# Fannovel16/ComfyUI-Frame-Interpolation

Hardware: AMD Instinct MI355X
Metric: interpolated frames/sec/GPU @1080p RIFE4.7 2x (higher is better)
Workload: dtype f32; 1 GPU; RIFE 4.7 2x, 1080x1920 synthetic frame-pair stream, 32 pairs/step/GPU resident in HBM (BASELINE.json configs[1]; SURVEY 8d config 2 clip: 33 frames torch.manual_seed(0) torch.rand); seeded random-init weights; new_frame_collective=none, launch=one process, one GPU

## Files before the change

### comfyui-frame-interpolation_amd/csrc/conv_mfma.hip

```cpp
#include "vfi_common.h"

#include <atomic>

#include <cstdlib>
#include <map>
#include <string>
#include <cstring>

namespace vfi {

typedef float f32x16 __attribute__((ext_vector_type(16)));
typedef float f32x4 __attribute__((ext_vector_type(4)));

template <int STRIDE, int TAPS, int MT, int NT, int WM, int WN, int CK, bool GROUPED, bool EXT>
__global__ __launch_bounds__(256) void conv_mfma_kernel(const ConvArgs a) {
    static_assert(WM * WN == 4, "4 waves per workgroup");
    static_assert(!GROUPED || (WN == 4 && NT == 1 && TAPS == 4), "grouped: one 2x2 tap group per wave column");
    static_assert(TAPS == 9 || TAPS == 4 || TAPS == 1, "tap rectangle 3x3 / 2x2 / 1x1");
    constexpr int KW = TAPS == 9 ? 3 : (TAPS == 4 ? 2 : 1);
    constexpr int SUBS = WM * MT;
    constexpr int SUBX = SUBS >= 2 ? 2 : 1;
    constexpr int SUBY = SUBS / SUBX;
    constexpr int TWO = SUBX * 8, THO = SUBY * 4;
    constexpr int TWI = STRIDE * (TWO - 1) + 3;
// ... 279 lines not shown
    static std::atomic<int> n_of[kMaxDevices];
    int dev = 0;
    if (hipGetDevice(&dev) != hipSuccess || dev < 0 || dev >= kMaxDevices) return 256;
    int n = n_of[dev].load(std::memory_order_relaxed);
    if (!n) {
        hipDeviceProp_t p;
        if (hipGetDeviceProperties(&p, dev) == hipSuccess) n = p.multiProcessorCount;
        if (n <= 0) n = 256;
        n_of[dev].store(n, std::memory_order_relaxed);
    }
    return n;
}

int conv_pick_variant(const ConvArgs& a, int stride, bool grouped) {
    const long px = (long)(a.split_ok ? a.N : 8) * a.Hout * a.Wout;
    if (!grouped && stride == 1 && a.ntaps == 4 && a.tapmask) return kConv2Base + (a.Cin_p % 16 == 0 ? 28 : 26);
    if (!grouped && stride == 2 && a.ntaps == 4) return kConv2Base + (a.Cout_p % 64 == 0 ? 21 : 20);
    if (!grouped && stride == 1 && a.ntaps != 9) {
        const bool big = px * (a.Cout_p / 32) >= 256L * 4 * n_cus_cached();
        if (a.ntaps == 1 && a.Cout_p % 64 == 0 && a.Cin_p % 32 == 0)
            return kConv2Base + (a.Cin_p >= 512 && a.Cout_p % 128 == 0 ? 24 : 23);
        if (a.Cout_p % 64 == 0) return kConv2Base + (a.ntaps == 4 ? (big ? 14 : 15) : (big ? 16 : 17));
        return kConv2Base + (a.ntaps == 4 ? 19 : 18);
    }
    const long cus = n_cus_cached();
    if (grouped) {
        if (a.out_mode == 1 && px >= 250000) return kConv2Base + 11;
        return a.Cin_p % 16 == 0 ? 13 : kConv2Base + 11;
    }
    const bool n3 = a.Cout_p % 96 == 0;
    const bool n2 = a.Cout_p % 64 == 0;
    (void)cus;
    if (stride == 2) {
        if (n2) return kConv2Base + 7;
        if (n3) return kConv2Base + 9;
        return 10;
    }
    if (a.split_ok && (n2 || n3) && px <= 6000) return kConv2Base + 29;
    if (n2) {
        const long big_px = option(kOptM2n2Px);
        if (a.Cout_p == 64 || (big_px >= 0 && px >= big_px)) return kConv2Base + 0;
        return kConv2Base + 2;
    }
    if (n3) return px >= 100000 || a.Cin_p % 16 ? kConv2Base + 3 : 4;
    return a.Cin_p % 16 == 0 && px < 20000 ? 4 : kConv2Base + 13;
}

int conv_launch(const ConvArgs& a, int stride, bool grouped, int variant, hipStream_t s,
                const char* trace_name) {
    if (variant < 0 && grouped && option(kOptGroupedVariant) >= 0) variant = (int)option(kOptGroupedVariant);
    if (variant < 0 && trace_name) variant = variant_override(trace_name);
    if (variant < 0) variant = conv_pick_variant(a, stride, grouped);
    const ConvVariant* vp = conv_variant_lookup(variant);
    VFI_REQUIRE(vp, "conv: bad variant %d", variant);
    const ConvVariant& v = *vp;
    VFI_REQUIRE(v.stride == stride && (v.grouped != 0) == grouped && v.taps == a.ntaps,
                "conv: variant %s does not match stride %d grouped %d taps %d", v.name, stride, (int)grouped,
                a.ntaps);
    VFI_REQUIRE(a.out_mode != 1 || (grouped && a.Cout % 4 == 0 && a.Cout / 4 <= 4 * (a.out_planes ? a.out_planes : 2)),
                "conv: out_mode 1 is for grouped convs whose pixel-shuffled channels fit the planar4 output");
    VFI_REQUIRE(a.out_mode != 2 || grouped, "conv: out_mode 2 is for grouped convs");
    VFI_REQUIRE(a.act != 3 || a.prelu, "conv: act 3 needs per-channel slopes");
    VFI_REQUIRE(a.Cin_p % 8 == 0 && a.Cout_p % 32 == 0 && a.in_cs >= a.Cin_p && a.in_cs % 4 == 0,
                "conv: bad channel padding Cin_p=%d Cout_p=%d in_cs=%d", a.Cin_p, a.Cout_p, a.in_cs);
    VFI_REQUIRE(((uintptr_t)a.in & 15) == 0 && ((uintptr_t)a.w & 15) == 0, "conv: unaligned pointers");
    const char* nm = trace_name ? trace_name : v.name;
// ... 108 lines not shown
```

### comfyui-frame-interpolation_amd/csrc/conv_mfma2.hip

```cpp
#include "vfi_common.h"

#include <atomic>
#include <cstdlib>
#include <map>
#include <mutex>
#include <utility>

namespace vfi {

typedef float f32x16 __attribute__((ext_vector_type(16)));
typedef float f32x4 __attribute__((ext_vector_type(4)));
typedef __attribute__((address_space(3))) void* lds_ptr_t;
typedef const __attribute__((address_space(1))) void* glb_ptr_t;

template <int STRIDE, int TAPS, int MT, int NT, int WM, int WN, int CK, bool GROUPED>
struct Conv2Geom {
    static constexpr int KW = TAPS == 9 ? 3 : (TAPS == 4 ? 2 : 1);
    static constexpr int SUBS = WM * MT;
    static constexpr int SUBX = SUBS >= 16 ? 4 : (SUBS >= 2 ? 2 : 1);
    static constexpr int SUBY = SUBS / SUBX;
    static constexpr int TWO = SUBX * 8, THO = SUBY * 4;
    static constexpr int PADLO = (TAPS == 9 || GROUPED) ? 1 : 0;
    static constexpr int SPAN = (TAPS == 9 || GROUPED) ? 3 : KW;
    static constexpr int TWI = STRIDE * (TWO - 1) + SPAN;
    static constexpr int THI = STRIDE * (THO - 1) + SPAN;
    static constexpr int NPIX = TWI * THI;
    static constexpr int Q = CK / 4;
    static constexpr int C8 = CK / 8;
    static constexpr int NA_INSTR = (NPIX * Q + 63) / 64;
    static constexpr int A_FLOATS = NA_INSTR * 256;
    static constexpr int NGRP = GROUPED ? 4 : 1;
    static constexpr int BN = GROUPED ? 32 : WN * NT * 32;
    static constexpr int NB_INSTR = NGRP * TAPS * C8 * (BN / 32);
    static constexpr int B_FLOATS = NB_INSTR * 256;
    static constexpr int BUF_FLOATS = A_FLOATS + B_FLOATS;
    static constexpr int LDS_BYTES = 2 * BUF_FLOATS * 4;
    static constexpr int NAW = (NA_INSTR + 3) / 4;
    static constexpr int NBW = (NB_INSTR + 3) / 4;
};

template <int STRIDE, int TAPS, int MT, int NT, int WM, int WN, int CK, bool GROUPED, bool EXT, bool MASKED = false>
__global__ __launch_bounds__(256) void conv_mfma2_kernel(const ConvArgs a) {
#if defined(__HIP_DEVICE_COMPILE__)
    using G = Conv2Geom<STRIDE, TAPS, MT, NT, WM, WN, CK, GROUPED>;
    static_assert(WM * WN == 4, "4 waves per workgroup");
    static_assert(!GROUPED || (WN == 4 && NT == 1 && TAPS == 4), "grouped: one 2x2 tap group per wave column");
    constexpr int KW = G::KW, SUBX = G::SUBX, TWO = G::TWO, THO = G::THO, TWI = G::TWI;
    constexpr int Q = G::Q, C8 = G::C8, BN = G::BN;

    extern __shared__ __attribute__((aligned(16))) float smem[];

    const int tid = threadIdx.x;
    const int lane = tid & 63;
    const int wave = __builtin_amdgcn_readfirstlane(tid >> 6);
    const int wm = wave / WN, wn = wave % WN;
    const int half = lane >> 5, l31 = lane & 31;

    const int g = GROUPED ? wn : 0;
    const int cob = blockIdx.y * BN;
    const int co0 = GROUPED ? cob : cob + wn * NT * 32;
    const int cin8 = a.Cin_p >> 3;
    const int tby = GROUPED ? (g >> 1) - 1 : a.tap_y0;
    const int tbx = GROUPED ? (g & 1) - 1 : a.tap_x0;

    const int tiles_per_img = a.tiles_x * a.tiles_y;
    const int T = a.N * tiles_per_img;
    const int pstr = a.in_plane ? 4 : a.in_cs;
    const int qstr = a.in_plane ? a.in_plane : 4;
    const int cadv = a.in_plane ? (CK / 4) * a.in_plane : CK;
    const int img_floats = a.in_plane ? (a.in_cs / 4) * a.in_plane : a.Hin * a.Win * a.in_cs;
    auto decode = [&](int tile, int& n, int& Y0, int& X0) {
        n = tile / tiles_per_img;
        const int trem = tile - n * tiles_per_img;
        const int ty = trem / a.tiles_x;
        Y0 = ty * THO;
        X0 = (trem - ty * a.tiles_x) * TWO;
    };
    auto make_avoff = [&](int Y0, int X0, int(&avoff)[G::NAW]) {
        const int iy0 = STRIDE * Y0 - G::PADLO, ix0 = STRIDE * X0 - G::PADLO;
#pragma unroll
        for (int i = 0; i < G::NAW; ++i) {
            const int j = wave + 4 * i;
            const int idx = j * 64 + lane;
            const int pix = idx / Q, q = idx - pix * Q;
            const int py = pix / TWI, px = pix - py * TWI;
            const int iy = iy0 + py, ix = ix0 + px;
            if (EXT && a.pad_mode) {
                const int cy = pad_index(iy, a.Hin, a.pad_mode), cx = pad_index(ix, a.Win, a.pad_mode);
                avoff[i] = pix < G::NPIX ? ((cy * a.Win + cx) * pstr + q * qstr) * 4 : (int)0x80000000;
            } else {
                const bool ok = pix < G::NPIX && iy >= 0 && iy < a.Hin && ix >= 0 && ix < a.Win;
                avoff[i] = ok ? ((iy * a.Win + ix) * pstr + q * qstr) * 4 : (int)0x80000000;
            }
        }
    };
    auto make_rsrc = [&](int n) {
        return __builtin_amdgcn_make_buffer_rsrc((void*)(a.in + (size_t)n * img_floats), 0, img_floats * 4, 0x00020000);
    };
    const unsigned tmask = MASKED ? a.tapmask[blockIdx.y] : 0xffffu;
    const int tapstride = cin8 * a.Cout_p * 8;
    const int c8stride = a.Cout_p * 8;
    const float* wsrc[G::NBW];
    bool wlive[G::NBW];
#pragma unroll
    for (int i = 0; i < G::NBW; ++i) {
        const int j = wave + 4 * i;
        const int sub = j % (BN / 32);
        const int c8 = (j / (BN / 32)) % C8;
        const int t = (j / (BN / 32) / C8) % TAPS;
        const int gg = j / (BN / 32) / C8 / TAPS;
        wsrc[i] = a.w + (size_t)(gg * TAPS + t) * tapstride + c8 * c8stride + (cob + sub * 32) * 8 + lane * 4;
        wlive[i] = !MASKED || ((tmask >> t) & 1u);
    }
    auto issue = [&](const __amdgpu_buffer_rsrc_t& rsrc, const int(&avoff)[G::NAW], int chunk, int buf) {
        float* abuf = smem + buf * G::BUF_FLOATS;
        float* bbuf = abuf + G::A_FLOATS;
        const int cbyte = chunk * cadv * 4;
#pragma unroll
        for (int i = 0; i < G::NAW; ++i) {
            const int j = wave + 4 * i;
            if (G::NA_INSTR % 4 == 0 || j < G::NA_INSTR)
                __builtin_amdgcn_raw_ptr_buffer_load_lds(rsrc, (lds_ptr_t)(abuf + j * 256), 16, avoff[i] + cbyte, 0, 0, 0);
        }
        const int wadv = chunk * C8 * c8stride;
#pragma unroll
        for (int i = 0; i < G::NBW; ++i) {
            const int j = wave + 4 * i;
            if ((G::NB_INSTR % 4 == 0 || j < G::NB_INSTR) && wlive[i])
                __builtin_amdgcn_global_load_lds((glb_ptr_t)(wsrc[i] + wadv), (lds_ptr_t)(bbuf + j * 256), 16, 0, 0);
        }
    };

    int abase[MT];
#pragma unroll
    for (int mt = 0; mt < MT; ++mt) {
        const int s = wm * MT + mt;
        const int sx = s % SUBX, sy = s / SUBX;
        const int oy = sy * 4 + (l31 >> 3), ox = sx * 8 + (l31 & 7);
        abase[mt] = ((STRIDE * oy + G::PADLO + tby) * TWI + STRIDE * ox + G::PADLO + tbx) * CK + half * 4;
    }
    const int bbase = G::A_FLOATS + (g * TAPS * C8 * BN + (co0 - cob) + l31) * 8 + half * 4;

    float bs[NT], bt[NT];
#pragma unroll
    for (int nt = 0; nt < NT; ++nt) {
        const int co = co0 + nt * 32 + l31;
        bs[nt] = a.bias[g * a.Cout_p + co];
        bt[nt] = a.beta ? a.beta[co] : 1.f;
    }

    int nchunks = a.Cin_p / CK, k0 = 0;
    float* const outp = a.out + (size_t)blockIdx.z * a.split_stride;
    if (a.ksplit > 1) {
        const int per = (nchunks + a.ksplit - 1) / a.ksplit;
        k0 = blockIdx.z * per;
        nchunks = nchunks - k0 < per ? nchunks - k0 : per;
    }

    int tile = blockIdx.x;
    if (tile >= T) return;
    int n, Y0, X0, avoff[G::NAW];
    decode(tile, n, Y0, X0);
    make_avoff(Y0, X0, avoff);
    __amdgpu_buffer_rsrc_t rsrc = make_rsrc(n);
    issue(rsrc, avoff, k0, 0);
    __syncthreads();
    int buf = 0;
    for (;;) {
        const int ntile = tile + gridDim.x;
        const bool has_next = ntile < T;
        int nn = 0, nY0 = 0, nX0 = 0, navoff[G::NAW];
        __amdgpu_buffer_rsrc_t nrsrc = rsrc;

        f32x16 acc[MT][NT];
#pragma unroll
        for (int mt = 0; mt < MT; ++mt)
#pragma unroll
            for (int nt = 0; nt < NT; ++nt)
#pragma unroll
                for (int r = 0; r < 16; ++r) acc[mt][nt][r] = 0.f;

        for (int k = 0; k < nchunks; ++k) {
            if (k + 1 < nchunks) {
                issue(rsrc, avoff, k0 + k + 1, buf ^ 1);
            } else if (has_next) {
                decode(ntile, nn, nY0, nX0);
                make_avoff(nY0, nX0, navoff);
                nrsrc = make_rsrc(nn);
                issue(nrsrc, navoff, k0, buf ^ 1);
            }
            const float* sb = smem + buf * G::BUF_FLOATS;
            constexpr int NS = TAPS * C8;
            f32x4 av[2][MT], bv[2][NT];
            auto frag = [&](int st, f32x4(&fa)[MT], f32x4(&fb)[NT]) {
                const int t = st / C8, c8 = st % C8;
                const int toff = ((t / KW) * TWI + (t % KW)) * CK + c8 * 8;
#pragma unroll
                for (int mt = 0; mt < MT; ++mt) fa[mt] = *(const f32x4*)&sb[abase[mt] + toff];
#pragma unroll
                for (int nt = 0; nt < NT; ++nt)
                    fb[nt] = *(const f32x4*)&sb[bbase + ((t * C8 + c8) * BN + nt * 32) * 8];
            };
            if constexpr (MASKED) {
                static_assert(!MASKED || TAPS == 4, "masked form: 2x2 taps");
                const unsigned m0 = tmask & 15u, m1 = m0 & (m0 - 1u), m2 = m1 & (m1 - 1u), m3 = m2 & (m2 - 1u);
                const int tl[4] = {m0 ? __builtin_ctz(m0) : 0, m1 ? __builtin_ctz(m1) : 0, m2 ? __builtin_ctz(m2) : 0, m3 ? __builtin_ctz(m3) : 0};
                const int ntl = __builtin_popcount(m0);
                auto run = [&](auto NTL) {
                    constexpr int n_ = decltype(NTL)::value * C8;
                    auto step_of = [&](int i) { return tl[i / C8] * C8 + i % C8; };
                    frag(step_of(0), av[0], bv[0]);
#pragma unroll
                    for (int i = 0; i < n_; ++i) {
                        __builtin_amdgcn_sched_barrier(0);
#pragma unroll
                        for (int j = 0; j < 4; ++j) {
#pragma unroll
                            for (int mt = 0; mt < MT; ++mt)
#pragma unroll
                                for (int nt = 0; nt < NT; ++nt)
                                    acc[mt][nt] = __builtin_amdgcn_mfma_f32_32x32x2f32(av[i & 1][mt][j], bv[i & 1][nt][j], acc[mt][nt], 0, 0, 0);
                            __builtin_amdgcn_sched_barrier(0);
                            if (j == 0 && i + 1 < n_) {
                                frag(step_of(i + 1), av[(i + 1) & 1], bv[(i + 1) & 1]);
                                __builtin_amdgcn_sched_barrier(0);
                            }
                        }
                    }
                };
                if (ntl == 1) run(std::integral_constant<int, 1>{});
                else if (ntl == 2) run(std::integral_constant<int, 2>{});
                else run(std::integral_constant<int, 4>{});
            } else {
            frag(0, av[0], bv[0]);
// ... 197 lines not shown
        float* p = nullptr;
        size_t n = 0;
        float* z = nullptr;
        int zn = 0;
    };
    static std::mutex mu;
    static std::map<std::pair<int, hipStream_t>, Ws> table;
    std::lock_guard<std::mutex> lock(mu);
    Ws& w = table[{dev, s}];
    if (w.n < floats) {
        w.p = nullptr, w.n = 0;
        VFI_CHECK_HIP(hipMalloc((void**)&w.p, floats * sizeof(float)));
        w.n = floats;
    }
    if (w.zn < cout_p) {
        w.z = nullptr, w.zn = 0;
        const int n = cout_p < 4096 ? 4096 : cout_p;
        VFI_CHECK_HIP(hipMalloc((void**)&w.z, n * sizeof(float)));
        VFI_CHECK_HIP(hipMemsetAsync(w.z, 0, n * sizeof(float), s));
        w.zn = n;
    }
    *ws = w.p, *zeros = w.z;
    return 0;
}

static int split_reduce(const ConvArgs& a, const float* ws, int ks, size_t slice, hipStream_t s) {
    TraceScope ts("conv_split_reduce", s);
    const long total = (long)a.N * a.Hout * a.Wout * a.Cout;
    hipLaunchKernelGGL(conv2_split_reduce_kernel, dim3((unsigned)((total + 255) / 256)), dim3(256), 0, s, a, ws, ks, (long)slice);
    VFI_CHECK_HIP(hipGetLastError());
    return 0;
}

template <int STRIDE, int TAPS, int MT, int NT, int WM, int WN, int CK, bool GROUPED, bool EXT, bool MASKED = false>
static int launch2_e(ConvArgs a, hipStream_t s, const char* name) {
    using G = Conv2Geom<STRIDE, TAPS, MT, NT, WM, WN, CK, GROUPED>;
    a.ksplit = 0, a.split_stride = 0;
    a.tiles_x = cdiv(a.Wout, G::TWO);
    a.tiles_y = cdiv(a.Hout, G::THO);
    VFI_REQUIRE(a.Cin_p % CK == 0, "conv2 %s: Cin_p=%d not a multiple of the K chunk %d", name, a.Cin_p, CK);
    VFI_REQUIRE(a.Cout_p % G::BN == 0, "conv2 %s: Cout_p=%d not a multiple of the N tile %d", name, a.Cout_p, G::BN);
    VFI_REQUIRE((long)a.Hin * a.Win * a.in_cs * 4 < 0x7fffffffL, "conv2 %s: image larger than 2 GiB", name);
    VFI_REQUIRE(!a.in_plane || a.in_plane >= a.Hin * a.Win * 4, "conv2 %s: bad plane stride", name);
    static std::atomic<int> occ_of[kMaxDevices];
    static std::atomic<int> cus_of[kMaxDevices];
    int dev = 0;
    VFI_CHECK_HIP(hipGetDevice(&dev));
    VFI_REQUIRE(dev >= 0 && dev < kMaxDevices, "conv2 %s: device index %d out of range", name, dev);
    int occ = occ_of[dev].load(std::memory_order_acquire);
    if (!occ) {
        VFI_CHECK_HIP(hipFuncSetAttribute(
            reinterpret_cast<const void*>(&conv_mfma2_kernel<STRIDE, TAPS, MT, NT, WM, WN, CK, GROUPED, EXT, MASKED>),
            hipFuncAttributeMaxDynamicSharedMemorySize, G::LDS_BYTES));
        int o = 0;
        VFI_CHECK_HIP(hipOccupancyMaxActiveBlocksPerMultiprocessor(
            &o, reinterpret_cast<const void*>(&conv_mfma2_kernel<STRIDE, TAPS, MT, NT, WM, WN, CK, GROUPED, EXT, MASKED>), 256,
            G::LDS_BYTES));
        hipDeviceProp_t p;
        VFI_CHECK_HIP(hipGetDeviceProperties(&p, dev));
        cus_of[dev].store(p.multiProcessorCount, std::memory_order_relaxed);
        occ = o < 1 ? 1 : o;
        occ_of[dev].store(occ, std::memory_order_release);
    }
    const int cus = cus_of[dev].load(std::memory_order_relaxed);
    const int T = a.N * a.tiles_x * a.tiles_y;
    const int ny = a.Cout_p / G::BN;
    int ks = 1;
    if (!GROUPED && !MASKED && a.out_mode == 0 && a.split_ok && split_enabled()) {
        const int nchunks = a.Cin_p / CK;
        const long wgs = (long)T * ny, want = 3L * cus * occ;
        const bool long_k = TAPS * nchunks >= 288, tiny = wgs * 8 <= (long)cus * occ && nchunks >= 16;
        if (wgs < (long)cus * occ && (long_k || tiny)) {
            ks = (int)((want + wgs - 1) / wgs);
            ks = ks > nchunks / 8 ? nchunks / 8 : ks;
            ks = ks > 16 ? 16 : ks;
            const int ks_traffic = TAPS * a.Cin_p / 576;
            ks = ks > ks_traffic ? ks_traffic : ks;
            ks = ks < 1 ? 1 : ks;
            const size_t slice = (size_t)a.N * a.Hout * a.Wout * a.Cout_p;
            while (ks > 1 && slice * ks * sizeof(float) > (256u << 20)) --ks;
            const int per = (nchunks + ks - 1) / ks;
            ks = (nchunks + per - 1) / per;
        }
    }
    if (ks > 1) {
        const size_t slice = (size_t)a.N * a.Hout * a.Wout * a.Cout_p;
        float *ws = nullptr, *zeros = nullptr;
        if (int rc = split_workspace(dev, s, slice * ks, a.Cout_p, &ws, &zeros)) return rc;
        ConvArgs p = a;
        p.out = ws, p.out_cs = a.Cout_p, p.bias = zeros, p.beta = nullptr, p.res = nullptr, p.res_cs = 0;
        p.act = 0, p.post_scale = 0.f, p.post_shift = 0.f, p.Cout = a.Cout_p;
        p.ksplit = ks, p.split_stride = (long)slice;
        {
            TraceScope ts(name, s);
            hipLaunchKernelGGL((conv_mfma2_kernel<STRIDE, TAPS, MT, NT, WM, WN, CK, GROUPED, EXT, MASKED>), dim3(T, ny, ks), dim3(256), G::LDS_BYTES, s, p);
            VFI_CHECK_HIP(hipGetLastError());
        }
        return split_reduce(a, ws, ks, slice, s);
    }
    int gx = (launch_cus(cus) * occ) / ny;
    if (gx < 1) gx = 1;
    if (gx > T || (long)T * ny < 4L * cus * occ) gx = T;
    if (MASKED) gx = T;
    dim3 grid(gx, ny);
    TraceScope ts(name, s);
    hipLaunchKernelGGL((conv_mfma2_kernel<STRIDE, TAPS, MT, NT, WM, WN, CK, GROUPED, EXT, MASKED>), grid, dim3(256), G::LDS_BYTES, s, a);
    VFI_CHECK_HIP(hipGetLastError());
    return 0;
}

template <int STRIDE, int TAPS, int MT, int NT, int WM, int WN, int CK>
static int launch2_masked(const ConvArgs& a, hipStream_t s, const char* name) {
    VFI_REQUIRE(a.tapmask && a.par_cout > 0 && a.par_cout % (WN * NT * 32) == 0 && a.Cout_p == 4 * a.par_cout && a.act <= 1 && !a.res && !a.beta && !a.in_plane,
                "conv2 %s: masked (up-sample x2 + 2x2) form needs 4 parity groups of a multiple of %d channels, act none / LeakyReLU", name, WN * NT * 32);
    return launch2_e<STRIDE, TAPS, MT, NT, WM, WN, CK, false, false, true>(a, s, name);
}

template <int STRIDE, int TAPS, int MT, int NT, int WM, int WN, int CK, bool GROUPED>
static int launch2_t(const ConvArgs& a, hipStream_t s, const char* name) {
    const bool ext = a.pad_mode || a.act >= 3 || a.post_scale != 0.f || a.out_mode == 2;
    return ext ? launch2_e<STRIDE, TAPS, MT, NT, WM, WN, CK, GROUPED, true>(a, s, name)
               : launch2_e<STRIDE, TAPS, MT, NT, WM, WN, CK, GROUPED, false>(a, s, name);
}

static const ConvVariant kVariants2[] = {
    {"d1_m2n2", 1, 9, 2, 2, 4, 1, 8, 0},
    {"d1_m2n3", 1, 9, 2, 3, 4, 1, 8, 0},
    {"d1_m1n2", 1, 9, 1, 2, 4, 1, 8, 0},
    {"d1_m1n3", 1, 9, 1, 3, 4, 1, 8, 0},
    {"d1_m2n2w22", 1, 9, 2, 2, 2, 2, 8, 0},
    {"d1_m4n2w22", 1, 9, 4, 2, 2, 2, 8, 0},
    {"d1_m2n2k16", 1, 9, 2, 2, 4, 1, 16, 0},
    {"d2_m1n2", 2, 9, 1, 2, 4, 1, 8, 0},
    {"d2_m2n2", 2, 9, 2, 2, 4, 1, 8, 0},
    {"d2_m1n3", 2, 9, 1, 3, 4, 1, 8, 0},
    {"d2_m2n1", 2, 9, 2, 1, 4, 1, 8, 0},
    {"dg_m4", 1, 4, 4, 1, 1, 4, 8, 1},
    {"dg_m8", 1, 4, 8, 1, 1, 4, 8, 1},
    {"d1_m2n1", 1, 9, 2, 1, 4, 1, 8, 0},
    {"d1t4_m2n2", 1, 4, 2, 2, 4, 1, 8, 0},
    {"d1t4_m1n2", 1, 4, 1, 2, 4, 1, 8, 0},
    {"d1t1_m2n2", 1, 1, 2, 2, 4, 1, 8, 0},
    {"d1t1_m1n2", 1, 1, 1, 2, 4, 1, 8, 0},
    {"d1t1_m2n1", 1, 1, 2, 1, 4, 1, 8, 0},
    {"d1t4_m2n1", 1, 4, 2, 1, 4, 1, 8, 0},
    {"d2t4_m2n1", 2, 4, 2, 1, 4, 1, 8, 0},
    {"d2t4_m1n2", 2, 4, 1, 2, 4, 1, 8, 0},
    {"d1_m4n2", 1, 9, 4, 2, 4, 1, 8, 0},
    {"d1t1_m1n2k32", 1, 1, 1, 2, 4, 1, 32, 0},
    {"d1t1_m2n2w22k32", 1, 1, 2, 2, 2, 2, 32, 0},
    {"d1t4_m2n2_up2", 1, 4, 2, 2, 4, 1, 8, 0},
    {"d1t4_m1n2_up2", 1, 4, 1, 2, 4, 1, 8, 0},
    {"d1t4_m2n2k16_up2", 1, 4, 2, 2, 4, 1, 16, 0},
    {"d1t4_m1n2k16_up2", 1, 4, 1, 2, 4, 1, 16, 0},
    {"d1_m1n1", 1, 9, 1, 1, 4, 1, 8, 0},
};
int conv2_num_variants() { return (int)(sizeof(kVariants2) / sizeof(kVariants2[0])); }
const ConvVariant& conv2_variant(int i) { return kVariants2[i]; }

int conv2_launch(const ConvArgs& a, int idx, hipStream_t s, const char* nm) {
    switch (idx) {
        case 0: return launch2_t<1, 9, 2, 2, 4, 1, 8, false>(a, s, nm);
        case 1: return launch2_t<1, 9, 2, 3, 4, 1, 8, false>(a, s, nm);
        case 2: return launch2_t<1, 9, 1, 2, 4, 1, 8, false>(a, s, nm);
        case 3: return launch2_t<1, 9, 1, 3, 4, 1, 8, false>(a, s, nm);
        case 4: return launch2_t<1, 9, 2, 2, 2, 2, 8, false>(a, s, nm);
        case 5: return launch2_t<1, 9, 4, 2, 2, 2, 8, false>(a, s, nm);
        case 6: return launch2_t<1, 9, 2, 2, 4, 1, 16, false>(a, s, nm);
        case 7: return launch2_t<2, 9, 1, 2, 4, 1, 8, false>(a, s, nm);
        case 8: return launch2_t<2, 9, 2, 2, 4, 1, 8, false>(a, s, nm);
        case 9: return launch2_t<2, 9, 1, 3, 4, 1, 8, false>(a, s, nm);
        case 10: return launch2_t<2, 9, 2, 1, 4, 1, 8, false>(a, s, nm);
        case 11: return launch2_t<1, 4, 4, 1, 1, 4, 8, true>(a, s, nm);
        case 12: return launch2_t<1, 4, 8, 1, 1, 4, 8, true>(a, s, nm);
        case 13: return launch2_t<1, 9, 2, 1, 4, 1, 8, false>(a, s, nm);
        case 14: return launch2_t<1, 4, 2, 2, 4, 1, 8, false>(a, s, nm);
        case 15: return launch2_t<1, 4, 1, 2, 4, 1, 8, false>(a, s, nm);
        case 16: return launch2_t<1, 1, 2, 2, 4, 1, 8, false>(a, s, nm);
        case 17: return launch2_t<1, 1, 1, 2, 4, 1, 8, false>(a, s, nm);
        case 18: return launch2_t<1, 1, 2, 1, 4, 1, 8, false>(a, s, nm);
        case 19: return launch2_t<1, 4, 2, 1, 4, 1, 8, false>(a, s, nm);
        case 20: return launch2_t<2, 4, 2, 1, 4, 1, 8, false>(a, s, nm);
        case 21: return launch2_t<2, 4, 1, 2, 4, 1, 8, false>(a, s, nm);
        case 22: return launch2_t<1, 9, 4, 2, 4, 1, 8, false>(a, s, nm);
        case 23: return launch2_t<1, 1, 1, 2, 4, 1, 32, false>(a, s, nm);
        case 24: return launch2_t<1, 1, 2, 2, 2, 2, 32, false>(a, s, nm);
        case 25: return launch2_masked<1, 4, 2, 2, 4, 1, 8>(a, s, nm);
        case 26: return launch2_masked<1, 4, 1, 2, 4, 1, 8>(a, s, nm);
        case 27: return launch2_masked<1, 4, 2, 2, 4, 1, 16>(a, s, nm);
        case 28: return launch2_masked<1, 4, 1, 2, 4, 1, 16>(a, s, nm);
        case 29: return launch2_t<1, 9, 1, 1, 4, 1, 8, false>(a, s, nm);
    }
    set_error("conv2: bad variant %d", idx);
    return -3;
}

}
```

### comfyui-frame-interpolation_amd/csrc/vfi_common.h

```cpp
#pragma once
#include <hip/hip_runtime.h>
#include <stdint.h>
#include <string>
#include <vector>

namespace vfi {

void set_error(const char* fmt, ...);
const char* get_error();

#define VFI_CHECK_HIP(expr)                                                                   \
    do {                                                                                      \
        hipError_t _e = (expr);                                                               \
        if (_e != hipSuccess) {                                                               \
            ::vfi::set_error("%s failed: %s (%s:%d)", #expr, hipGetErrorString(_e), __FILE__, \
                             __LINE__);                                                       \
            return -1;                                                                        \
        }                                                                                     \
    } while (0)

#define VFI_REQUIRE(cond, ...)          \
    do {                                \
        if (!(cond)) {                  \
            ::vfi::set_error(__VA_ARGS__); \
// ... 70 lines not shown
    const float* res;
    float* out;
    int N, Hin, Win, in_cs;
    int Hout, Wout, out_cs, res_cs;
    int Cin_p, Cout_p, Cout;
    int ntaps;
    int act;
    float slope;
    int tiles_x, tiles_y;
    int tap_y0, tap_x0;
    int in_plane;
    int out_mode;
    int out_planes;
    int pad_mode;
    const float* prelu;
    float post_scale, post_shift;
    int split_ok;
    const unsigned char* tapmask;
    int par_cout;
    int ksplit;
    long split_stride;
};

struct ConvVariant {
    const char* name;
    int stride, taps, mt, nt, wm, wn, ck, grouped;
};
constexpr int kConv2Base = 32;
int conv_num_variants();
const ConvVariant& conv_variant(int i);
int conv2_num_variants();
const ConvVariant& conv2_variant(int i);
int conv2_launch(const ConvArgs& a, int idx, hipStream_t s, const char* trace_name);
const ConvVariant* conv_variant_lookup(int id);
int conv_pick_variant(const ConvArgs& a, int stride, bool grouped);
int conv_launch(const ConvArgs& a, int stride, bool grouped, int variant, hipStream_t s,
                const char* trace_name);

void pack_conv3x3(const float* w_oihw, const float* bias, int Cout, int Cin, int Cin_p,
                  int Cout_p, std::vector<float>& wp, std::vector<float>& bp);
void pack_deconv4x4(const float* w_iohw, const float* bias, int Cin, int Cout, int Cin_p,
                    int Cout_p, std::vector<float>& wp, std::vector<float>& bp);
void conv3x3_taps(ConvArgs& a);

void pack_wino3x3(const float* w_oihw, int Cout, int Cin, const int* chan_map, int Cin_p, int Cout_p, std::vector<float>& wp);
void pack_deconv_as_conv3x3(const float* w_iohw, const float* bias, int Cin, int LO, std::vector<float>& w3, std::vector<float>& b3);
bool conv_wino_eligible(const ConvArgs& a);
int conv_wino_mode(int set);
int conv_wino_launch(const ConvArgs& a, int variant, hipStream_t s, const char* trace_name);
void deconv4x4_taps(ConvArgs& a);

int conv_naive_launch(const float* in, const float* w_oihw_dev, const float* bias_dev,
                      const float* beta_dev, float* out, int N, int H, int W, int Cin, int in_cs,
                      int Cout, int stride, int act, float slope, hipStream_t s);

}
```

Measured before the change: 853.6 frames/s.

## Keep stride-2 conv weights resident in LDS with 8-wave workgroups

Adds a resident-weights variant of the MFMA conv kernel for stride-2 3x3 convs. Each workgroup has 8 waves and loads the whole weight slice for its output-channel block into LDS once, using up to 160 KiB. After that it streams only input tiles through a double buffer, so it no longer reloads weights on every K chunk. The picker uses this variant whenever split-K is off and the weights fit. In exchange, each workgroup takes a large LDS footprint and occupancy drops.

New measurement: 859.3 frames/s, median of 6. About the same (+0.7%).

```diff
diff --git a/comfyui-frame-interpolation_amd/csrc/conv_mfma.hip b/comfyui-frame-interpolation_amd/csrc/conv_mfma.hip
--- a/comfyui-frame-interpolation_amd/csrc/conv_mfma.hip
+++ b/comfyui-frame-interpolation_amd/csrc/conv_mfma.hip
@@ -335,6 +335,10 @@
     const bool n2 = a.Cout_p % 64 == 0;
     (void)cus;
     if (stride == 2) {
+        if (!a.split_ok) {
+            const int bn = n2 ? 64 : (n3 ? 96 : 0);
+            if (bn && conv2_res_lds_bytes(a.Cin_p, bn) <= kConv2ResLds) return kConv2Base + (bn == 64 ? 30 : 31);
+        }
         if (n2) return kConv2Base + 7;
         if (n3) return kConv2Base + 9;
         return 10;
diff --git a/comfyui-frame-interpolation_amd/csrc/conv_mfma2.hip b/comfyui-frame-interpolation_amd/csrc/conv_mfma2.hip
--- a/comfyui-frame-interpolation_amd/csrc/conv_mfma2.hip
+++ b/comfyui-frame-interpolation_amd/csrc/conv_mfma2.hip
@@ -15,6 +15,7 @@
 
 template <int STRIDE, int TAPS, int MT, int NT, int WM, int WN, int CK, bool GROUPED>
 struct Conv2Geom {
+    static constexpr int NW = WM * WN;
     static constexpr int KW = TAPS == 9 ? 3 : (TAPS == 4 ? 2 : 1);
     static constexpr int SUBS = WM * MT;
     static constexpr int SUBX = SUBS >= 16 ? 4 : (SUBS >= 2 ? 2 : 1);
@@ -35,18 +36,19 @@
     static constexpr int B_FLOATS = NB_INSTR * 256;
     static constexpr int BUF_FLOATS = A_FLOATS + B_FLOATS;
     static constexpr int LDS_BYTES = 2 * BUF_FLOATS * 4;
-    static constexpr int NAW = (NA_INSTR + 3) / 4;
-    static constexpr int NBW = (NB_INSTR + 3) / 4;
+    static constexpr int NAW = (NA_INSTR + NW - 1) / NW;
+    static constexpr int NBW = (NB_INSTR + NW - 1) / NW;
 };
 
-template <int STRIDE, int TAPS, int MT, int NT, int WM, int WN, int CK, bool GROUPED, bool EXT, bool MASKED = false>
-__global__ __launch_bounds__(256) void conv_mfma2_kernel(const ConvArgs a) {
+template <int STRIDE, int TAPS, int MT, int NT, int WM, int WN, int CK, bool GROUPED, bool EXT, bool MASKED = false, bool RESW = false>
+__global__ __launch_bounds__(64 * WM * WN) void conv_mfma2_kernel(const ConvArgs a) {
 #if defined(__HIP_DEVICE_COMPILE__)
     using G = Conv2Geom<STRIDE, TAPS, MT, NT, WM, WN, CK, GROUPED>;
-    static_assert(WM * WN == 4, "4 waves per workgroup");
+    static_assert(WM * WN == 4 || (RESW && WM * WN == 8), "4 waves per workgroup (8 with resident weights)");
     static_assert(!GROUPED || (WN == 4 && NT == 1 && TAPS == 4), "grouped: one 2x2 tap group per wave column");
+    static_assert(!RESW || (!GROUPED && !MASKED && CK == 8), "resident weights: plain convs, 8-channel K chunks");
     constexpr int KW = G::KW, SUBX = G::SUBX, TWO = G::TWO, THO = G::THO, TWI = G::TWI;
-    constexpr int Q = G::Q, C8 = G::C8, BN = G::BN;
+    constexpr int Q = G::Q, C8 = G::C8, BN = G::BN, NW = G::NW;
 
     extern __shared__ __attribute__((aligned(16))) float smem[];
 
@@ -76,11 +78,37 @@
         Y0 = ty * THO;
         X0 = (trem - ty * a.tiles_x) * TWO;
     };
+    int ppy[G::NAW], ppx[G::NAW], pq[G::NAW];
+    if constexpr (RESW) {
+#pragma unroll
+        for (int i = 0; i < G::NAW; ++i) {
+            const int idx = (wave + NW * i) * 64 + lane;
+            const int pix = idx / Q, q = idx - pix * Q;
+            const int py = pix / TWI;
+            ppy[i] = pix < G::NPIX ? py : -(1 << 24);
+            ppx[i] = pix - py * TWI;
+            pq[i] = q;
+        }
+    }
     auto make_avoff = [&](int Y0, int X0, int(&avoff)[G::NAW]) {
         const int iy0 = STRIDE * Y0 - G::PADLO, ix0 = STRIDE * X0 - G::PADLO;
+        if constexpr (RESW) {
+#pragma unroll
+            for (int i = 0; i < G::NAW; ++i) {
+                const int iy = iy0 + ppy[i], ix = ix0 + ppx[i];
+                if (EXT && a.pad_mode) {
+                    const int cy = pad_index(iy, a.Hin, a.pad_mode), cx = pad_index(ix, a.Win, a.pad_mode);
+                    avoff[i] = ppy[i] >= 0 ? ((cy * a.Win + cx) * pstr + pq[i] * qstr) * 4 : (int)0x80000000;
+                } else {
+                    const bool ok = (unsigned)iy < (unsigned)a.Hin && (unsigned)ix < (unsigned)a.Win;
+                    avoff[i] = ok ? ((iy * a.Win + ix) * pstr + pq[i] * qstr) * 4 : (int)0x80000000;
+                }
+            }
+            return;
+        }
 #pragma unroll
         for (int i = 0; i < G::NAW; ++i) {
-            const int j = wave + 4 * i;
+            const int j = wave + NW * i;
             const int idx = j * 64 + lane;
             const int pix = idx / Q, q = idx - pix * Q;
             const int py = pix / TWI, px = pix - py * TWI;
@@ -104,7 +132,7 @@
     bool wlive[G::NBW];
 #pragma unroll
     for (int i = 0; i < G::NBW; ++i) {
-        const int j = wave + 4 * i;
+        const int j = wave + NW * i;
         const int sub = j % (BN / 32);
         const int c8 = (j / (BN / 32)) % C8;
         const int t = (j / (BN / 32) / C8) % TAPS;
@@ -113,20 +141,21 @@
         wlive[i] = !MASKED || ((tmask >> t) & 1u);
     }
     auto issue = [&](const __amdgpu_buffer_rsrc_t& rsrc, const int(&avoff)[G::NAW], int chunk, int buf) {
-        float* abuf = smem + buf * G::BUF_FLOATS;
+        float* abuf = smem + buf * (RESW ? G::A_FLOATS : G::BUF_FLOATS);
         float* bbuf = abuf + G::A_FLOATS;
         const int cbyte = chunk * cadv * 4;
 #pragma unroll
         for (int i = 0; i < G::NAW; ++i) {
-            const int j = wave + 4 * i;
-            if (G::NA_INSTR % 4 == 0 || j < G::NA_INSTR)
+            const int j = wave + NW * i;
+            if (G::NA_INSTR % NW == 0 || j < G::NA_INSTR)
                 __builtin_amdgcn_raw_ptr_buffer_load_lds(rsrc, (lds_ptr_t)(abuf + j * 256), 16, avoff[i] + cbyte, 0, 0, 0);
         }
+        if constexpr (RESW) return;
         const int wadv = chunk * C8 * c8stride;
 #pragma unroll
         for (int i = 0; i < G::NBW; ++i) {
-            const int j = wave + 4 * i;
-            if ((G::NB_INSTR % 4 == 0 || j < G::NB_INSTR) && wlive[i])
+            const int j = wave + NW * i;
+            if ((G::NB_INSTR % NW == 0 || j < G::NB_INSTR) && wlive[i])
                 __builtin_amdgcn_global_load_lds((glb_ptr_t)(wsrc[i] + wadv), (lds_ptr_t)(bbuf + j * 256), 16, 0, 0);
         }
     };
@@ -139,7 +168,7 @@
         const int oy = sy * 4 + (l31 >> 3), ox = sx * 8 + (l31 & 7);
         abase[mt] = ((STRIDE * oy + G::PADLO + tby) * TWI + STRIDE * ox + G::PADLO + tbx) * CK + half * 4;
     }
-    const int bbase = G::A_FLOATS + (g * TAPS * C8 * BN + (co0 - cob) + l31) * 8 + half * 4;
+    const int bbase = (RESW ? 0 : G::A_FLOATS) + (g * TAPS * C8 * BN + (co0 - cob) + l31) * 8 + half * 4;
 
     float bs[NT], bt[NT];
 #pragma unroll
@@ -159,6 +188,16 @@
 
     int tile = blockIdx.x;
     if (tile >= T) return;
+    if constexpr (RESW) {
+        float* bres = smem + 2 * G::A_FLOATS;
+        const int npieces = nchunks * G::NB_INSTR;
+        for (int j = wave; j < npieces; j += NW) {
+            const int kc = j / G::NB_INSTR, jj = j - kc * G::NB_INSTR;
+            const int sub = jj % (BN / 32), c8 = (jj / (BN / 32)) % C8, t = jj / (BN / 32) / C8;
+            const float* src = a.w + (size_t)t * tapstride + ((k0 + kc) * C8 + c8) * c8stride + (cob + sub * 32) * 8 + lane * 4;
+            __builtin_amdgcn_global_load_lds((glb_ptr_t)src, (lds_ptr_t)(bres + j * 256), 16, 0, 0);
+        }
+    }
     int n, Y0, X0, avoff[G::NAW];
     decode(tile, n, Y0, X0);
     make_avoff(Y0, X0, avoff);
@@ -189,7 +228,8 @@
                 nrsrc = make_rsrc(nn);
                 issue(nrsrc, navoff, k0, buf ^ 1);
             }
-            const float* sb = smem + buf * G::BUF_FLOATS;
+            const float* sb = smem + buf * (RESW ? G::A_FLOATS : G::BUF_FLOATS);
+            const float* sw = RESW ? smem + 2 * G::A_FLOATS + k * G::B_FLOATS : sb;
             constexpr int NS = TAPS * C8;
             f32x4 av[2][MT], bv[2][NT];
             auto frag = [&](int st, f32x4(&fa)[MT], f32x4(&fb)[NT]) {
@@ -199,7 +239,7 @@
                 for (int mt = 0; mt < MT; ++mt) fa[mt] = *(const f32x4*)&sb[abase[mt] + toff];
 #pragma unroll
                 for (int nt = 0; nt < NT; ++nt)
-                    fb[nt] = *(const f32x4*)&sb[bbase + ((t * C8 + c8) * BN + nt * 32) * 8];
+                    fb[nt] = *(const f32x4*)&sw[bbase + ((t * C8 + c8) * BN + nt * 32) * 8];
             };
             if constexpr (MASKED) {
                 static_assert(!MASKED || TAPS == 4, "masked form: 2x2 taps");
@@ -463,9 +503,11 @@
     return 0;
 }
 
-template <int STRIDE, int TAPS, int MT, int NT, int WM, int WN, int CK, bool GROUPED, bool EXT, bool MASKED = false>
+template <int STRIDE, int TAPS, int MT, int NT, int WM, int WN, int CK, bool GROUPED, bool EXT, bool MASKED = false, bool RESW = false>
 static int launch2_e(ConvArgs a, hipStream_t s, const char* name) {
     using G = Conv2Geom<STRIDE, TAPS, MT, NT, WM, WN, CK, GROUPED>;
+    constexpr int NTH = 64 * G::NW;
+    auto kern = &conv_mfma2_kernel<STRIDE, TAPS, MT, NT, WM, WN, CK, GROUPED, EXT, MASKED, RESW>;
     a.ksplit = 0, a.split_stride = 0;
     a.tiles_x = cdiv(a.Wout, G::TWO);
     a.tiles_y = cdiv(a.Hout, G::THO);
@@ -473,6 +515,8 @@
     VFI_REQUIRE(a.Cout_p % G::BN == 0, "conv2 %s: Cout_p=%d not a multiple of the N tile %d", name, a.Cout_p, G::BN);
     VFI_REQUIRE((long)a.Hin * a.Win * a.in_cs * 4 < 0x7fffffffL, "conv2 %s: image larger than 2 GiB", name);
     VFI_REQUIRE(!a.in_plane || a.in_plane >= a.Hin * a.Win * 4, "conv2 %s: bad plane stride", name);
+    const int lds = RESW ? (2 * G::A_FLOATS + (a.Cin_p / CK) * G::B_FLOATS) * 4 : G::LDS_BYTES;
+    VFI_REQUIRE(lds <= kConv2ResLds, "conv2 %s: Cin_p=%d needs %d B of LDS for resident weights", name, a.Cin_p, lds);
     static std::atomic<int> occ_of[kMaxDevices];
     static std::atomic<int> cus_of[kMaxDevices];
     int dev = 0;
@@ -480,13 +524,10 @@
     VFI_REQUIRE(dev >= 0 && dev < kMaxDevices, "conv2 %s: device index %d out of range", name, dev);
     int occ = occ_of[dev].load(std::memory_order_acquire);
     if (!occ) {
-        VFI_CHECK_HIP(hipFuncSetAttribute(
-            reinterpret_cast<const void*>(&conv_mfma2_kernel<STRIDE, TAPS, MT, NT, WM, WN, CK, GROUPED, EXT, MASKED>),
-            hipFuncAttributeMaxDynamicSharedMemorySize, G::LDS_BYTES));
+        const int lds_max = RESW ? kConv2ResLds : G::LDS_BYTES;
+        VFI_CHECK_HIP(hipFuncSetAttribute(reinterpret_cast<const void*>(kern), hipFuncAttributeMaxDynamicSharedMemorySize, lds_max));
         int o = 0;
-        VFI_CHECK_HIP(hipOccupancyMaxActiveBlocksPerMultiprocessor(
-            &o, reinterpret_cast<const void*>(&conv_mfma2_kernel<STRIDE, TAPS, MT, NT, WM, WN, CK, GROUPED, EXT, MASKED>), 256,
-            G::LDS_BYTES));
+        VFI_CHECK_HIP(hipOccupancyMaxActiveBlocksPerMultiprocessor(&o, reinterpret_cast<const void*>(kern), NTH, lds_max));
         hipDeviceProp_t p;
         VFI_CHECK_HIP(hipGetDeviceProperties(&p, dev));
         cus_of[dev].store(p.multiProcessorCount, std::memory_order_relaxed);
@@ -524,7 +565,7 @@
         p.ksplit = ks, p.split_stride = (long)slice;
         {
             TraceScope ts(name, s);
-            hipLaunchKernelGGL((conv_mfma2_kernel<STRIDE, TAPS, MT, NT, WM, WN, CK, GROUPED, EXT, MASKED>), dim3(T, ny, ks), dim3(256), G::LDS_BYTES, s, p);
+            hipLaunchKernelGGL(kern, dim3(T, ny, ks), dim3(NTH), lds, s, p);
             VFI_CHECK_HIP(hipGetLastError());
         }
         return split_reduce(a, ws, ks, slice, s);
@@ -535,7 +576,7 @@
     if (MASKED) gx = T;
     dim3 grid(gx, ny);
     TraceScope ts(name, s);
-    hipLaunchKernelGGL((conv_mfma2_kernel<STRIDE, TAPS, MT, NT, WM, WN, CK, GROUPED, EXT, MASKED>), grid, dim3(256), G::LDS_BYTES, s, a);
+    hipLaunchKernelGGL(kern, grid, dim3(NTH), lds, s, a);
     VFI_CHECK_HIP(hipGetLastError());
     return 0;
 }
@@ -547,11 +588,16 @@
     return launch2_e<STRIDE, TAPS, MT, NT, WM, WN, CK, false, false, true>(a, s, name);
 }
 
-template <int STRIDE, int TAPS, int MT, int NT, int WM, int WN, int CK, bool GROUPED>
+template <int STRIDE, int TAPS, int MT, int NT, int WM, int WN, int CK, bool GROUPED, bool RESW = false>
 static int launch2_t(const ConvArgs& a, hipStream_t s, const char* name) {
     const bool ext = a.pad_mode || a.act >= 3 || a.post_scale != 0.f || a.out_mode == 2;
-    return ext ? launch2_e<STRIDE, TAPS, MT, NT, WM, WN, CK, GROUPED, true>(a, s, name)
-               : launch2_e<STRIDE, TAPS, MT, NT, WM, WN, CK, GROUPED, false>(a, s, name);
+    return ext ? launch2_e<STRIDE, TAPS, MT, NT, WM, WN, CK, GROUPED, true, false, RESW>(a, s, name)
+               : launch2_e<STRIDE, TAPS, MT, NT, WM, WN, CK, GROUPED, false, false, RESW>(a, s, name);
+}
+
+int conv2_res_lds_bytes(int cin_p, int bn) {
+    using G = Conv2Geom<2, 9, 1, 2, 8, 1, 8, false>;
+    return (2 * G::A_FLOATS + 9 * cin_p * bn) * 4;
 }
 
 static const ConvVariant kVariants2[] = {
@@ -585,6 +631,8 @@
     {"d1t4_m2n2k16_up2", 1, 4, 2, 2, 4, 1, 16, 0},
     {"d1t4_m1n2k16_up2", 1, 4, 1, 2, 4, 1, 16, 0},
     {"d1_m1n1", 1, 9, 1, 1, 4, 1, 8, 0},
+    {"d2r_m1n2", 2, 9, 1, 2, 8, 1, 8, 0},
+    {"d2r_m1n3", 2, 9, 1, 3, 8, 1, 8, 0},
 };
 int conv2_num_variants() { return (int)(sizeof(kVariants2) / sizeof(kVariants2[0])); }
 const ConvVariant& conv2_variant(int i) { return kVariants2[i]; }
@@ -621,6 +669,8 @@
         case 27: return launch2_masked<1, 4, 2, 2, 4, 1, 16>(a, s, nm);
         case 28: return launch2_masked<1, 4, 1, 2, 4, 1, 16>(a, s, nm);
         case 29: return launch2_t<1, 9, 1, 1, 4, 1, 8, false>(a, s, nm);
+        case 30: return launch2_t<2, 9, 1, 2, 8, 1, 8, false, true>(a, s, nm);
+        case 31: return launch2_t<2, 9, 1, 3, 8, 1, 8, false, true>(a, s, nm);
     }
     set_error("conv2: bad variant %d", idx);
     return -3;
diff --git a/comfyui-frame-interpolation_amd/csrc/vfi_common.h b/comfyui-frame-interpolation_amd/csrc/vfi_common.h
--- a/comfyui-frame-interpolation_amd/csrc/vfi_common.h
+++ b/comfyui-frame-interpolation_amd/csrc/vfi_common.h
@@ -126,6 +126,8 @@
 int conv2_num_variants();
 const ConvVariant& conv2_variant(int i);
 int conv2_launch(const ConvArgs& a, int idx, hipStream_t s, const char* trace_name);
+constexpr int kConv2ResLds = 160 * 1024;
+int conv2_res_lds_bytes(int cin_p, int bn);
 const ConvVariant* conv_variant_lookup(int id);
 int conv_pick_variant(const ConvArgs& a, int stride, bool grouped);
 int conv_launch(const ConvArgs& a, int stride, bool grouped, int variant, hipStream_t s,
```

## Add persistent weight-resident stride-2 3x3 conv kernel for large 64-channel layers

Applied to the files above, without the earlier changes.

Adds a new persistent 512-thread kernel for stride-2 3x3 convolutions. It keeps the whole weight slice for a Cout block resident in LDS and loops over output tiles, double-buffering activation chunks via buffer_load_lds with explicit waitcnt scheduling. The picker routes large stride-2 layers with Cout_p==64 to it when the LDS footprint fits under 160KB, and falls back to the existing variant otherwise. This aims to remove repeated weight reloads and per-tile launch overhead, in exchange for heavy LDS use and lower occupancy.

Result: no change. 859.1 frames/s before, 863.0 frames/s after, median of 6 (+0.5%).

```diff
diff --git a/comfyui-frame-interpolation_amd/csrc/conv_mfma.hip b/comfyui-frame-interpolation_amd/csrc/conv_mfma.hip
--- a/comfyui-frame-interpolation_amd/csrc/conv_mfma.hip
+++ b/comfyui-frame-interpolation_amd/csrc/conv_mfma.hip
@@ -335,6 +335,7 @@
     const bool n2 = a.Cout_p % 64 == 0;
     (void)cus;
     if (stride == 2) {
+        if (n2 && px >= 500000 && a.Cout_p == 64 && s2res_eligible(a, 64, 160 * 1024)) return kConv2Base + 30;
         if (n2) return kConv2Base + 7;
         if (n3) return kConv2Base + 9;
         return 10;
diff --git a/comfyui-frame-interpolation_amd/csrc/conv_mfma2.hip b/comfyui-frame-interpolation_amd/csrc/conv_mfma2.hip
--- a/comfyui-frame-interpolation_amd/csrc/conv_mfma2.hip
+++ b/comfyui-frame-interpolation_amd/csrc/conv_mfma2.hip
@@ -585,6 +585,8 @@
     {"d1t4_m2n2k16_up2", 1, 4, 2, 2, 4, 1, 16, 0},
     {"d1t4_m1n2k16_up2", 1, 4, 1, 2, 4, 1, 16, 0},
     {"d1_m1n1", 1, 9, 1, 1, 4, 1, 8, 0},
+    {"d2r_m1n2", 2, 9, 1, 2, 8, 1, 8, 0},
+    {"d2r_m1n3", 2, 9, 1, 3, 8, 1, 8, 0},
 };
 int conv2_num_variants() { return (int)(sizeof(kVariants2) / sizeof(kVariants2[0])); }
 const ConvVariant& conv2_variant(int i) { return kVariants2[i]; }
@@ -621,6 +623,13 @@
         case 27: return launch2_masked<1, 4, 2, 2, 4, 1, 16>(a, s, nm);
         case 28: return launch2_masked<1, 4, 1, 2, 4, 1, 16>(a, s, nm);
         case 29: return launch2_t<1, 9, 1, 1, 4, 1, 8, false>(a, s, nm);
+        case 30:
+        case 31: {
+            bool ran = false;
+            if (int rc = conv_s2res_launch(a, idx == 30 ? 2 : 3, s, nm, &ran)) return rc;
+            if (ran) return 0;
+            return idx == 30 ? launch2_t<2, 9, 1, 2, 4, 1, 8, false>(a, s, nm) : launch2_t<2, 9, 1, 3, 4, 1, 8, false>(a, s, nm);
+        }
     }
     set_error("conv2: bad variant %d", idx);
     return -3;
diff --git a/comfyui-frame-interpolation_amd/csrc/conv_s2res.hip b/comfyui-frame-interpolation_amd/csrc/conv_s2res.hip
--- /dev/null
+++ b/comfyui-frame-interpolation_amd/csrc/conv_s2res.hip
@@ -0,0 +1,267 @@
+#include "vfi_common.h"
+
+#include <atomic>
+
+namespace vfi {
+
+typedef float f32x16 __attribute__((ext_vector_type(16)));
+typedef float f32x4 __attribute__((ext_vector_type(4)));
+typedef __attribute__((address_space(3))) void* lds_ptr_t;
+typedef const __attribute__((address_space(1))) void* glb_ptr_t;
+
+namespace {
+
+struct S2Res {
+    static constexpr int WAVES = 8;
+    static constexpr int SUBW = 8, SUBH = 4;
+    static constexpr int SUBX = 4, SUBY = 2;
+    static constexpr int TWO = SUBX * SUBW, THO = SUBY * SUBH;
+    static constexpr int PW = 2 * (SUBW - 1) + 3, PH = 2 * (SUBH - 1) + 3;
+    static constexpr int NPIX = PW * PH;
+    static constexpr int CK = 8;
+    static constexpr int NA = (NPIX * (CK / 4) + 63) / 64;
+    static constexpr int A_FLOATS = NA * 256;
+    static constexpr int ACT_FLOATS = WAVES * 2 * A_FLOATS;
+};
+
+constexpr int s2res_waitcnt(int vm, int lgkm) { return (vm & 15) | (7 << 4) | ((lgkm & 15) << 8) | ((vm >> 4) << 14); }
+
+}
+
+size_t s2res_lds_bytes(int cin_p, int bn) { return ((size_t)9 * cin_p * bn + S2Res::ACT_FLOATS) * sizeof(float); }
+
+template <int NT>
+__global__ __launch_bounds__(512) void conv_s2res_kernel(const ConvArgs a) {
+#if defined(__HIP_DEVICE_COMPILE__)
+    using G = S2Res;
+    constexpr int BN = NT * 32, PW = G::PW, CK = G::CK;
+    extern __shared__ __attribute__((aligned(16))) float smem[];
+
+    const int tid = threadIdx.x;
+    const int lane = tid & 63;
+    const int wave = __builtin_amdgcn_readfirstlane(tid >> 6);
+    const int half = lane >> 5, l31 = lane & 31;
+    const int sx = wave & (G::SUBX - 1), sy = wave / G::SUBX;
+    const int cob = blockIdx.y * BN;
+    const int cin8 = a.Cin_p >> 3;
+    const int w_floats = 9 * cin8 * BN * 8;
+    float* const abuf0 = smem + w_floats + wave * 2 * G::A_FLOATS;
+
+    const int tiles_per_img = a.tiles_x * a.tiles_y;
+    const int T = a.N * tiles_per_img;
+    const int pstr = a.in_plane ? 4 : a.in_cs;
+    const int qstr = a.in_plane ? a.in_plane : 4;
+    const int cadv = a.in_plane ? (CK / 4) * a.in_plane : CK;
+    const int img_floats = a.in_plane ? (a.in_cs / 4) * a.in_plane : a.Hin * a.Win * a.in_cs;
+    auto decode = [&](int tile, int& n, int& Y0, int& X0) {
+        n = tile / tiles_per_img;
+        const int trem = tile - n * tiles_per_img;
+        const int ty = trem / a.tiles_x;
+        Y0 = ty * G::THO + sy * G::SUBH;
+        X0 = (trem - ty * a.tiles_x) * G::TWO + sx * G::SUBW;
+    };
+    auto make_avoff = [&](int Y0, int X0, int(&avoff)[G::NA]) {
+        const int iy0 = 2 * Y0 - 1, ix0 = 2 * X0 - 1;
+#pragma unroll
+        for (int i = 0; i < G::NA; ++i) {
+            const int idx = i * 64 + lane;
+            const int pix = idx >> 1, q = idx & 1;
+            const int py = pix / PW, px = pix - py * PW;
+            const int iy = iy0 + py, ix = ix0 + px;
+            const bool ok = pix < G::NPIX && iy >= 0 && iy < a.Hin && ix >= 0 && ix < a.Win;
+            avoff[i] = ok ? ((iy * a.Win + ix) * pstr + q * qstr) * 4 : (int)0x80000000;
+        }
+    };
+    auto make_rsrc = [&](int n) {
+        return __builtin_amdgcn_make_buffer_rsrc((void*)(a.in + (size_t)n * img_floats), 0, img_floats * 4, 0x00020000);
+    };
+    auto issue = [&](const __amdgpu_buffer_rsrc_t& rsrc, const int(&avoff)[G::NA], int chunk, int buf) {
+        float* ab = abuf0 + buf * G::A_FLOATS;
+        const int cbyte = chunk * cadv * 4;
+#pragma unroll
+        for (int i = 0; i < G::NA; ++i)
+            __builtin_amdgcn_raw_ptr_buffer_load_lds(rsrc, (lds_ptr_t)(ab + i * 256), 16, avoff[i] + cbyte, 0, 0, 0);
+    };
+
+    {
+        const int npieces = 9 * cin8 * NT;
+        const int c8stride = a.Cout_p * 8;
+        for (int j = wave; j < npieces; j += G::WAVES) {
+            const int row = j / NT, sub = j - row * NT;
+            const float* src = a.w + (size_t)row * c8stride + (cob + sub * 32) * 8 + (lane & 31) * 8 + (lane >> 5) * 4;
+            __builtin_amdgcn_global_load_lds((glb_ptr_t)src, (lds_ptr_t)(smem + j * 256), 16, 0, 0);
+        }
+    }
+
+    const int abase = ((2 * (l31 >> 3)) * PW + 2 * (l31 & 7)) * CK + half * 4;
+    const int bbase = half * 128 + l31 * 4;
+    const int tapstr = cin8 * BN * 8;
+
+    float bs[NT], bt[NT];
+#pragma unroll
+    for (int nt = 0; nt < NT; ++nt) {
+        const int co = cob + nt * 32 + l31;
+        bs[nt] = a.bias[co];
+        bt[nt] = a.beta ? a.beta[co] : 1.f;
+    }
+    const int nchunks = a.Cin_p / CK;
+
+    int dtile = blockIdx.x, dk = 0, dbuf = 0, dn, dY0, dX0, davoff[G::NA];
+    decode(dtile, dn, dY0, dX0);
+    make_avoff(dY0, dX0, davoff);
+    __amdgpu_buffer_rsrc_t drsrc = make_rsrc(dn);
+    auto issue_next = [&]() {
+        if (dtile < T) {
+            issue(drsrc, davoff, dk, dbuf);
+            if (++dk == nchunks) {
+                dk = 0;
+                dtile += gridDim.x;
+                if (dtile < T) {
+                    decode(dtile, dn, dY0, dX0);
+                    make_avoff(dY0, dX0, davoff);
+                    drsrc = make_rsrc(dn);
+                }
+            }
+        }
+        dbuf ^= 1;
+    };
+    issue_next();
+    issue_next();
+    __syncthreads();
+
+    f32x4 av[2], bv[2][NT];
+    auto frag = [&](int buf, int k, int t, f32x4& fa, f32x4(&fb)[NT]) {
+        const float* sa = abuf0 + buf * G::A_FLOATS + abase;
+        const float* sw = smem + k * (BN * 8) + bbase;
+        fa = *(const f32x4*)&sa[((t / 3) * PW + (t % 3)) * CK];
+#pragma unroll
+        for (int nt = 0; nt < NT; ++nt) fb[nt] = *(const f32x4*)&sw[t * tapstr + nt * 256];
+    };
+    frag(0, 0, 0, av[0], bv[0]);
+    int buf = 0;
+    for (int tile = blockIdx.x; tile < T; tile += gridDim.x) {
+        f32x16 acc[NT];
+#pragma unroll
+        for (int nt = 0; nt < NT; ++nt)
+#pragma unroll
+            for (int r = 0; r < 16; ++r) acc[nt][r] = 0.f;
+
+        for (int k = 0; k < nchunks; ++k) {
+#pragma unroll
+            for (int t = 0; t < 9; ++t) {
+                __builtin_amdgcn_sched_barrier(0);
+#pragma unroll
+                for (int j = 0; j < 4; ++j) {
+#pragma unroll
+                    for (int nt = 0; nt < NT; ++nt)
+                        acc[nt] = __builtin_amdgcn_mfma_f32_32x32x2f32(av[t & 1][j], bv[t & 1][nt][j], acc[nt], 0, 0, 0);
+                    __builtin_amdgcn_sched_barrier(0);
+                    if (j == 0) {
+                        if (t + 1 < 9) {
+                            frag(buf, k, t + 1, av[(t + 1) & 1], bv[(t + 1) & 1]);
+                        } else {
+                            __builtin_amdgcn_s_waitcnt(s2res_waitcnt(0, 15));
+                            __builtin_amdgcn_sched_barrier(0);
+                            frag(buf ^ 1, k + 1 < nchunks ? k + 1 : 0, 0, av[1], bv[1]);
+                            __builtin_amdgcn_sched_barrier(0);
+                            issue_next();
+                        }
+                        __builtin_amdgcn_sched_barrier(0);
+                    }
+                }
+            }
+            av[0] = av[1];
+#pragma unroll
+            for (int nt = 0; nt < NT; ++nt) bv[0][nt] = bv[1][nt];
+            buf ^= 1;
+        }
+
+        int n, Y0, X0;
+        decode(tile, n, Y0, X0);
+        {
+            const int xstr = a.out_cs, ystr = a.Wout * a.out_cs;
+            const bool interior = Y0 + G::SUBH <= a.Hout && X0 + G::SUBW <= a.Wout;
+            const bool unif01 = a.act == 0 || (a.act == 1 && a.slope >= 0.f && a.slope <= 1.f);
+            const float uslope = a.act == 1 ? a.slope : 1.0f;
+            const int ox0 = X0 + 4 * half;
+#pragma unroll
+            for (int nt = 0; nt < NT; ++nt) {
+                const int co = cob + nt * 32 + l31;
+                if (co < a.Cout) {
+                    float* ob = a.out + ((size_t)(n * a.Hout + Y0) * a.Wout + ox0) * a.out_cs + co;
+                    if (unif01 && interior) {
+#pragma unroll
+                        for (int r = 0; r < 16; ++r) {
+                            const float v = (acc[nt][r] + bs[nt]) * bt[nt];
+                            ob[(r >> 2) * ystr + (r & 3) * xstr] = fmaxf(v, v * uslope);
+                        }
+                    } else {
+                        const float sl = a.act == 0 ? 1.0f : a.slope;
+#pragma unroll
+                        for (int r = 0; r < 16; ++r) {
+                            float v = (acc[nt][r] + bs[nt]) * bt[nt];
+                            v = v > 0.f ? v : v * sl;
+                            if (interior || (Y0 + (r >> 2) < a.Hout && ox0 + (r & 3) < a.Wout)) ob[(r >> 2) * ystr + (r & 3) * xstr] = v;
+                        }
+                    }
+                }
+            }
+        }
+    }
+#endif
+}
+
+bool s2res_eligible(const ConvArgs& a, int bn, size_t lds_limit) {
+    if (a.ntaps != 9 || a.tap_y0 != -1 || a.tap_x0 != -1) return false;
+    if (a.pad_mode || a.act >= 2 || a.post_scale != 0.f || a.out_mode != 0 || a.res || a.tapmask) return false;
+    if (a.Hin % 2 || a.Win % 2 || a.Hout * 2 != a.Hin || a.Wout * 2 != a.Win) return false;
+    if (a.Cin_p % S2Res::CK || a.Cout_p % bn) return false;
+    return s2res_lds_bytes(a.Cin_p, bn) <= lds_limit;
+}
+
+template <int NT>
+static int launch_s2res(ConvArgs a, hipStream_t s, const char* name, bool* ran) {
+    constexpr int BN = NT * 32;
+    *ran = false;
+    static std::atomic<int> lds_of[kMaxDevices];
+    static std::atomic<int> cus_of[kMaxDevices];
+    int dev = 0;
+    VFI_CHECK_HIP(hipGetDevice(&dev));
+    VFI_REQUIRE(dev >= 0 && dev < kMaxDevices, "conv2 %s: device index %d out of range", name, dev);
+    int lim = lds_of[dev].load(std::memory_order_acquire);
+    if (!lim) {
+        hipDeviceProp_t p;
+        VFI_CHECK_HIP(hipGetDeviceProperties(&p, dev));
+        int optin = (int)p.sharedMemPerBlock;
+        int v = 0;
+        if (hipDeviceGetAttribute(&v, hipDeviceAttributeSharedMemPerBlockOptin, dev) == hipSuccess && v > optin) optin = v;
+        (void)hipGetLastError();
+        if ((int)p.maxSharedMemoryPerMultiProcessor > optin) optin = (int)p.maxSharedMemoryPerMultiProcessor;
+        VFI_CHECK_HIP(hipFuncSetAttribute(reinterpret_cast<const void*>(&conv_s2res_kernel<NT>), hipFuncAttributeMaxDynamicSharedMemorySize, optin));
+        cus_of[dev].store(p.multiProcessorCount, std::memory_order_relaxed);
+        lim = optin;
+        lds_of[dev].store(lim, std::memory_order_release);
+    }
+    if (!s2res_eligible(a, BN, (size_t)lim)) return 0;
+    a.ksplit = 0, a.split_stride = 0;
+    a.tiles_x = cdiv(a.Wout, S2Res::TWO);
+    a.tiles_y = cdiv(a.Hout, S2Res::THO);
+    VFI_REQUIRE((long)a.Hin * a.Win * a.in_cs * 4 < 0x7fffffffL, "conv2 %s: image larger than 2 GiB", name);
+    VFI_REQUIRE(!a.in_plane || a.in_plane >= a.Hin * a.Win * 4, "conv2 %s: bad plane stride", name);
+    const int T = a.N * a.tiles_x * a.tiles_y;
+    const int ny = a.Cout_p / BN;
+    int gx = launch_cus(cus_of[dev].load(std::memory_order_relaxed)) / ny;
+    if (gx < 1) gx = 1;
+    if (gx > T) gx = T;
+    TraceScope ts(name, s);
+    hipLaunchKernelGGL((conv_s2res_kernel<NT>), dim3(gx, ny), dim3(512), s2res_lds_bytes(a.Cin_p, BN), s, a);
+    VFI_CHECK_HIP(hipGetLastError());
+    *ran = true;
+    return 0;
+}
+
+int conv_s2res_launch(const ConvArgs& a, int nt, hipStream_t s, const char* name, bool* ran) {
+    return nt == 3 ? launch_s2res<3>(a, s, name, ran) : launch_s2res<2>(a, s, name, ran);
+}
+
+}
diff --git a/comfyui-frame-interpolation_amd/csrc/vfi_common.h b/comfyui-frame-interpolation_amd/csrc/vfi_common.h
--- a/comfyui-frame-interpolation_amd/csrc/vfi_common.h
+++ b/comfyui-frame-interpolation_amd/csrc/vfi_common.h
@@ -126,6 +126,9 @@
 int conv2_num_variants();
 const ConvVariant& conv2_variant(int i);
 int conv2_launch(const ConvArgs& a, int idx, hipStream_t s, const char* trace_name);
+size_t s2res_lds_bytes(int cin_p, int bn);
+bool s2res_eligible(const ConvArgs& a, int bn, size_t lds_limit);
+int conv_s2res_launch(const ConvArgs& a, int nt, hipStream_t s, const char* trace_name, bool* ran);
 const ConvVariant* conv_variant_lookup(int id);
 int conv_pick_variant(const ConvArgs& a, int stride, bool grouped);
 int conv_launch(const ConvArgs& a, int stride, bool grouped, int variant, hipStream_t s,
```
